# oramasearch/oramacore

Hardware: NVIDIA H100
Metric: hybrid_search_qps_at_recall10_ge_0.99_1Mx768 (higher is better)
Workload: dtype f32

## Files before the change

oramacore_b200/csrc/bm25.cuh:

```cuda
#pragma once
#include "oc_common.cuh"

namespace oc {

#ifndef OC_BM25_TILE_ROWS
#define OC_BM25_TILE_ROWS 8192
#endif
constexpr uint32_t BM25_TILE = OC_BM25_TILE_ROWS;
#ifndef OC_BM25_THREADS
#define OC_BM25_THREADS 256
#endif
constexpr uint32_t BM25_THREADS = OC_BM25_THREADS;
constexpr uint32_t BM25_CHUNK = BM25_THREADS * 4;

struct PostingRaw {
    uint32_t row;
    uint16_t tf, len;
};
struct Posting {
    uint32_t row;
    float ntf;
};

struct TermDesc {
// ... 951 lines not shown
    if (s3 != 0.f) t3_consider(s3, row + 3u, tau, tau_f, s_cnt, tbuf, cap);
}
__device__ __forceinline__ uint32_t f32_ne0_mask(const float x) {
    uint32_t r;
    asm("set.neu.u32.f32 %0, %1, 0f00000000;" : "=r"(r) : "f"(x));
    return r;
}
template <uint32_t ND, uint32_t STRIDE>
__device__ __forceinline__ void t3_scan(const float4 *d0, const float4 *d1, const float4 *d2, const float4 *d3,
                                        const uint32_t *touched, const bool any_list, const bool pos, const uint32_t row0, const uint32_t tid,
                                        const unsigned long long tau, const float tau_f, uint32_t *s_cnt, uint64_t *tbuf,
                                        const uint32_t cap, uint32_t &matched, float &lmax, float &lmin) {
    constexpr uint32_t F4 = BM25_TILE / 4 / STRIDE;
    constexpr uint32_t FB = (ND <= 2 && F4 >= 4) ? 2 : 1;
    constexpr uint32_t NB = F4 / FB;
    static_assert(F4 >= 2 && NB % 2 == 0, "tile size");
    const float4 *dp[4] = {d0, d1, d2, d3};
    const uint32_t *tw = touched + (tid >> 3);
    const uint32_t tsh = (tid & 7u) * 4u;
    float4 ca[ND][FB], cb[ND][FB];
    auto load = [&](float4 (&c)[ND][FB], const uint32_t h) {
#pragma unroll
        for (uint32_t u = 0; u < FB; u++)
#pragma unroll
            for (uint32_t d = 0; d < ND; d++) c[d][u] = __ldg(dp[d] + tid + (h * FB + u) * STRIDE);
    };
    auto fold = [&](const float4 (&c)[ND][FB], const uint32_t h) {
#pragma unroll
        for (uint32_t u = 0; u < FB; u++) {
            const uint32_t i = tid + (h * FB + u) * STRIDE;
            float sv[4] = {c[0][u].x, c[0][u].y, c[0][u].z, c[0][u].w};
#pragma unroll
            for (uint32_t d = 1; d < ND; d++) {
                sv[0] = __fadd_rn(sv[0], c[d][u].x); sv[1] = __fadd_rn(sv[1], c[d][u].y);
                sv[2] = __fadd_rn(sv[2], c[d][u].z); sv[3] = __fadd_rn(sv[3], c[d][u].w);
            }
            if (any_list) {
                const uint32_t bits = (tw[(h * FB + u) * (STRIDE / 8)] >> tsh) & 0xfu;
                if (bits) {
#pragma unroll
                    for (int k = 0; k < 4; k++) sv[k] = ((bits >> k) & 1u) ? 0.f : sv[k];
                }
            }
            matched -= f32_ne0_mask(sv[0]) + f32_ne0_mask(sv[1]) + f32_ne0_mask(sv[2]) + f32_ne0_mask(sv[3]);
            const float m4 = fmaxf(fmaxf(sv[0], sv[1]), fmaxf(sv[2], sv[3]));
            lmax = fmaxf(lmax, m4);
            if (!pos) lmin = fminf(lmin, fminf(fminf(sv[0], sv[1]), fminf(sv[2], sv[3])));
            if (m4 >= tau_f) t3_consider4(sv[0], sv[1], sv[2], sv[3], row0 + i * 4u, tau, tau_f, s_cnt, tbuf, cap);
        }
    };
    load(ca, 0);
#pragma unroll 1
    for (uint32_t h = 0; h < NB; h += 2) {
        load(cb, h + 1);
        fold(ca, h);
        if (h + 2 < NB) load(ca, h + 2);
        fold(cb, h + 1);
    }
}

__device__ __forceinline__ float t3_dense_ub(const ItemTok *tab) {
    float ub = 0.f;
#pragma unroll
    for (uint32_t j = 0; j < BM25_FLAT_TOK; j++)
        if (tab[j].n && (tab[j].flags & TD_DENSE)) ub = __fadd_rn(ub, __uint_as_float(tab[j].bound));
    return ub;
}
template <uint32_t STRIDE>
__device__ __noinline__ uint32_t t3_count(const ItemTok *tab, const uint32_t *touched, const bool any_list, const uint32_t n_tiles,
                                          const uint32_t tile, const uint32_t tid) {
    constexpr uint32_t W = BM25_TILE / 32;
    const uint32_t *bp[BM25_FLAT_TOK];
#pragma unroll
    for (uint32_t j = 0; j < BM25_FLAT_TOK; j++)
        bp[j] = (tab[j].n && (tab[j].flags & TD_DENSE))
                    ? bm25_dense_bits(reinterpret_cast<const float *>(tab[j].ptr) - size_t(tile) * BM25_TILE, n_tiles) + size_t(tile) * W
                    : nullptr;
    uint32_t m = 0;
#pragma unroll 2
    for (uint32_t w = tid; w < W; w += STRIDE) {
        uint32_t u = 0;
#pragma unroll
        for (uint32_t j = 0; j < BM25_FLAT_TOK; j++) if (bp[j]) u |= __ldg(bp[j] + w);
        if (any_list) u &= ~touched[w];
        m += __popc(u);
    }
    return m;
}

__global__ void __launch_bounds__(BM25_THREADS, 1024 / BM25_THREADS) bm25_tile3_kernel(const Bm25Params p, const ItemTok *flat, unsigned int *work_counter) {
    constexpr uint32_t W = BM25_TILE / 32;
    extern __shared__ __align__(16) uint8_t smem[];
    uint32_t *touched = reinterpret_cast<uint32_t *>(smem);
    uint32_t *bm = touched + W;
    uint64_t *tbuf = reinterpret_cast<uint64_t *>(bm + BM25_FLAT_TOK * W);
    __shared__ uint32_t s_cnt2[2], s_matched2[2];
    __shared__ unsigned int s_maxo2[2], s_mino2[2];
    __shared__ ItemTok s_tab[2][BM25_FLAT_TOK];
    __shared__ uint32_t s_item_cur, s_item_next;
    __shared__ uint32_t s_dense[2];
    __shared__ unsigned long long s_tau2[2];

    const uint32_t tid = threadIdx.x;
    const float kp1 = __fadd_rn(p.k, 1.0f);
    const uint32_t n_items = p.n_tiles * p.n_queries;
    const uint32_t *okbits = p.row_ok_bits;
// ... 130 lines not shown
            c = p.n_keep;
            if (tid == 0) atomicMax(p.tau + q, (unsigned long long)tbuf[p.n_keep - 1]);
        }
        for (uint32_t i = tid; i < c; i += BM25_THREADS) {
            const uint64_t key = tbuf[i];
            p.cand_key[slot_base * p.n_keep + i] = key;
            p.cand_ft[slot_base * p.n_keep + i] = key_score(key);
        }
        if (tid == 0) {
            p.cand_cnt[slot_base] = c;
            p.tile_count[slot_base] = s_matched2[par];
            p.tile_max[slot_base] = f32_unordered(s_maxo2[par]);
            p.tile_min[slot_base] = f32_unordered(s_mino2[par]);
        }
        if (tid < BM25_FLAT_TOK) s_tab[par ^ 1u][tid] = nx;
        if (tid == 0) { s_item_cur = next; s_item_next = next2; s_tau2[par ^ 1u] = tau_next; }
    }
    if (tid == 0 && p.dense_stat && s_dense[0]) { atomicAdd(p.dense_stat, s_dense[0]); atomicAdd(p.dense_stat + 1, s_dense[1]); }
}

constexpr uint32_t BW_WARPS = 6, BW_CAP = 256;
struct __align__(16) WarpScratch {
    uint32_t touched[BM25_TILE / 32];
    uint32_t bm[BM25_FLAT_TOK * (BM25_TILE / 32)];
    uint64_t tbuf[BW_CAP];
    ItemTok tab[BM25_FLAT_TOK];
    uint32_t cnt, dense_items, dense_skipped, pad;
};
__device__ __noinline__ unsigned long long warp_keep_top(uint64_t *buf, const uint32_t count, const uint32_t n, const uint32_t lane) {
    constexpr uint32_t PER = BW_CAP / 32;
    unsigned long long k[PER];
#pragma unroll
    for (uint32_t u = 0; u < PER; u++) k[u] = lane + 32u * u < count ? buf[lane + 32u * u] : 0ull;
    __syncwarp();
    unsigned long long mine = 0ull, last = 0ull;
    for (uint32_t r = 0; r < n; r++) {
        unsigned long long m = k[0];
#pragma unroll
        for (uint32_t u = 1; u < PER; u++) m = k[u] > m ? k[u] : m;
        for (int o = 16; o > 0; o >>= 1) {
            const unsigned long long om = __shfl_xor_sync(0xffffffffu, m, o);
            m = om > m ? om : m;
        }
        last = m;
        if (m == 0ull) break;
        if (lane == r) mine = m;
#pragma unroll
        for (uint32_t u = 0; u < PER; u++) if (k[u] == m) k[u] = 0ull;
    }
    if (lane < n) buf[lane] = mine;
    __syncwarp();
    return last;
}
__global__ void __launch_bounds__(BW_WARPS * 32, 5) bm25_warp_kernel(const Bm25Params p, const ItemTok *flat, unsigned int *work_counter) {
    constexpr uint32_t W = BM25_TILE / 32;
    extern __shared__ __align__(16) uint8_t smem[];
    const uint32_t lane = threadIdx.x & 31u;
    WarpScratch &ws = reinterpret_cast<WarpScratch *>(smem)[threadIdx.x >> 5];
    uint32_t *touched = ws.touched, *bm = ws.bm;
    const ItemTok *tab = ws.tab;
    const float kp1 = __fadd_rn(p.k, 1.0f);
    const uint32_t n_items = p.n_tiles * p.n_queries;
    const uint32_t *okbits = p.row_ok_bits;

    for (uint32_t i = lane; i < W; i += 32) touched[i] = 0u;
    for (uint32_t i = lane; i < BM25_FLAT_TOK * W; i += 32) bm[i] = 0u;
    if (lane == 0) { ws.cnt = 0u; ws.dense_items = 0u; ws.dense_skipped = 0u; }
    uint32_t item = 0, next = 0;
    if (lane == 0) { item = atomicAdd(work_counter, 1u); next = atomicAdd(work_counter, 1u); }
    item = __shfl_sync(0xffffffffu, item, 0); next = __shfl_sync(0xffffffffu, next, 0);
    ItemTok cur{};
    if (item < n_items && lane < BM25_FLAT_TOK) cur = flat[size_t(item) * BM25_FLAT_TOK + lane];
    unsigned long long tau_next = 0ull;
    if (item < n_items) tau_next = __ldcg(p.tau + item % p.n_queries);

    while (item < n_items) {
        uint32_t next2 = 0;
        if (lane == 0) next2 = atomicAdd(work_counter, 1u);
        const uint32_t tile = item / p.n_queries, q = item % p.n_queries;
        const uint32_t row0 = tile * BM25_TILE;
        if (lane < BM25_FLAT_TOK) ws.tab[lane] = cur;
        ItemTok nx{};
        if (next < n_items && lane < BM25_FLAT_TOK) nx = flat[size_t(next) * BM25_FLAT_TOK + lane];
        unsigned long long tau = __shfl_sync(0xffffffffu, tau_next, 0);
        if (next < n_items) tau_next = __ldcg(p.tau + next % p.n_queries);
        __syncwarp();

        const float4 *d0 = nullptr, *d1 = nullptr, *d2 = nullptr, *d3 = nullptr;
        uint32_t nd = 0, n_list = 0;
        bool pos = p.k >= 0.f;
#pragma unroll
        for (uint32_t j = 0; j < BM25_FLAT_TOK; j++) {
            const uint32_t n = tab[j].n;
            if (n == 0) continue;
            pos = pos && tab[j].w >= 0.f && tab[j].idf >= 0.f;
            if (tab[j].flags & TD_DENSE) {
                const float4 *dp = reinterpret_cast<const float4 *>(tab[j].ptr);
                if (nd == 0) d0 = dp; else if (nd == 1) d1 = dp; else if (nd == 2) d2 = dp; else d3 = dp;
                nd++;
            } else n_list++;
        }
        const bool any_list = n_list != 0;
        const bool use_bm = n_list > 1 || okbits != nullptr;
        uint32_t matched;
        float lmax, lmin;
        for (;;) {
            const float tau_f = tau ? key_score(tau) : -INFINITY;
            matched = 0; lmax = 0.f; lmin = 0.f;
            if (any_list && (nd || use_bm)) {
#pragma unroll 1
                for (uint32_t j = 0; j < BM25_FLAT_TOK; j++) {
                    const uint32_t n = tab[j].n;
                    if (n == 0 || (tab[j].flags & TD_DENSE)) continue;
                    const uint2 *pp = reinterpret_cast<const uint2 *>(tab[j].ptr);
                    for (uint32_t pi = lane; pi < n; pi += 32) {
                        const uint32_t row = __ldg(&pp[pi].x);
                        if (okbits && !((__ldg(okbits + (row >> 5)) >> (row & 31u)) & 1u)) continue;
                        const uint32_t l = row - row0, bit = 1u << (l & 31u);
                        if (nd) atomicOr(&touched[l >> 5], bit);
                        if (use_bm) atomicOr(&bm[j * W + (l >> 5)], bit);
                    }
                }
                __syncwarp();
            }
            const bool skip = nd && pos && t3_dense_ub(tab) < tau_f;
            if (nd && lane == 0) { ws.dense_items++; ws.dense_skipped += skip; }
            if (skip) matched += t3_count<32>(tab, touched, any_list, p.n_tiles, tile, lane);
            else switch (nd) {
                case 0: break;
                case 1: t3_scan<1, 32>(d0, d1, d2, d3, touched, any_list, pos, row0, lane, tau, tau_f, &ws.cnt, ws.tbuf, BW_CAP, matched, lmax, lmin); break;
                case 2: t3_scan<2, 32>(d0, d1, d2, d3, touched, any_list, pos, row0, lane, tau, tau_f, &ws.cnt, ws.tbuf, BW_CAP, matched, lmax, lmin); break;
                case 3: t3_scan<3, 32>(d0, d1, d2, d3, touched, any_list, pos, row0, lane, tau, tau_f, &ws.cnt, ws.tbuf, BW_CAP, matched, lmax, lmin); break;
                default: t3_scan<4, 32>(d0, d1, d2, d3, touched, any_list, pos, row0, lane, tau, tau_f, &ws.cnt, ws.tbuf, BW_CAP, matched, lmax, lmin); break;
            }
            if (any_list) {
#pragma unroll 1
                for (uint32_t j = 0; j < BM25_FLAT_TOK; j++) {
                    const uint32_t n = tab[j].n;
                    if (n == 0 || (tab[j].flags & TD_DENSE)) continue;
                    const uint2 *pp = reinterpret_cast<const uint2 *>(tab[j].ptr);
                    for (uint32_t pi = lane; pi < n; pi += 32) {
                        const uint2 rec = __ldg(pp + pi);
                        const uint32_t l = rec.x - row0, w = l >> 5, bit = 1u << (l & 31u);
                        if (use_bm) {
                            if (!(bm[j * W + w] & bit)) continue;
                            uint32_t earlier = 0;
                            for (uint32_t jj = 0; jj < j; jj++) earlier |= bm[jj * W + w];
                            if (earlier & bit) continue;
                        }
                        const float s = t3_fold(tab, bm, j, rec, l, p.k, kp1);
                        if (s != 0.f) {
                            matched++;
                            lmax = fmaxf(lmax, s);
                            lmin = fminf(lmin, s);
                            t3_consider(s, rec.x, tau, tau_f, &ws.cnt, ws.tbuf, BW_CAP);
                        }
                    }
                }
            }
            __syncwarp();
            if (any_list) {
                if (nd) for (uint32_t i = lane; i < W; i += 32) touched[i] = 0u;
                if (use_bm) for (uint32_t i = lane; i < BM25_FLAT_TOK * W; i += 32) bm[i] = 0u;
            }
            if (ws.cnt <= BW_CAP) break;
            const unsigned long long kth = warp_keep_top(ws.tbuf, BW_CAP, p.n_keep, lane) - 1ull;
            tau = kth > tau ? kth : tau;
            if (lane == 0) ws.cnt = 0u;
            __syncwarp();
        }
        matched = __reduce_add_sync(0xffffffffu, matched);
        for (int o = 16; o > 0; o >>= 1) {
            lmax = fmaxf(lmax, __shfl_xor_sync(0xffffffffu, lmax, o));
            lmin = fminf(lmin, __shfl_xor_sync(0xffffffffu, lmin, o));
        }
        const size_t slot_base = (size_t(q) * p.n_tiles + tile);
        uint32_t c = ws.cnt;
        if (c >= p.n_keep && c > 0) {
            const unsigned long long kth = warp_keep_top(ws.tbuf, c, p.n_keep, lane);
            c = p.n_keep;
            if (lane == 0) atomicMax(p.tau + q, kth);
        }
        for (uint32_t i = lane; i < c; i += 32) {
            const uint64_t key = ws.tbuf[i];
            p.cand_key[slot_base * p.n_keep + i] = key;
            p.cand_ft[slot_base * p.n_keep + i] = key_score(key);
        }
        __syncwarp();
        if (lane == 0) {
            p.cand_cnt[slot_base] = c;
            p.tile_count[slot_base] = matched;
            p.tile_max[slot_base] = lmax;
            p.tile_min[slot_base] = lmin;
            ws.cnt = 0u;
        }
        if (lane < BM25_FLAT_TOK && nx.n) {
            const char *pf = reinterpret_cast<const char *>(nx.ptr);
            const uint32_t bytes = (nx.flags & TD_DENSE) ? 1024u : min(nx.n * 8u, 1024u);
            for (uint32_t o = 0; o < bytes; o += 128u) asm volatile("prefetch.global.L1 [%0];" ::"l"(pf + o));
        }
        cur = nx;
        item = next;
        next = __shfl_sync(0xffffffffu, next2, 0);
        __syncwarp();
    }
    if (lane == 0 && p.dense_stat && ws.dense_items) { atomicAdd(p.dense_stat, ws.dense_items); atomicAdd(p.dense_stat + 1, ws.dense_skipped); }
}

struct PointParams {
    const TermDesc *terms; const TokenDesc *tokens; const QueryDesc *queries;
    uint32_t n_queries, v_stride;
    const uint32_t *v_row;
    const uint32_t *row_ok_bits;
    float k;
    int threshold;
    float *v_ft; uint8_t *v_present;
    const uint32_t *q_ok_slot;
    uint64_t ok_words;
};
__device__ __forceinline__ bool posting_find(const TermDesc &td, uint32_t row, uint32_t *payload) {
    const uint2 *pp = reinterpret_cast<const uint2 *>(td.ptr);
    uint32_t lo = 0, hi = td.len;
    while (lo < hi) { const uint32_t m = (lo + hi) >> 1; if (__ldg(&pp[m].x) < row) lo = m + 1; else hi = m; }
    if (lo < td.len) { const uint2 r = __ldg(pp + lo); if (r.x == row) { *payload = r.y; return true; } }
    return false;
}
__global__ void __launch_bounds__(256) bm25_point_kernel(const PointParams p) {
    const uint32_t wid = (blockIdx.x * blockDim.x + threadIdx.x) / 32, lane = threadIdx.x & 31;
    if (wid >= p.n_queries * p.v_stride) return;
    const uint32_t q = wid / p.v_stride;
    const uint32_t r = p.v_row[wid];
    const QueryDesc qd = p.queries[q];
    const float kp1 = __fadd_rn(p.k, 1.0f);
    float score = 0.f;
    uint32_t mask = 0;
    bool ok = r != 0xffffffffu;
    if (ok && p.row_ok_bits) ok = (row_ok_of(p.row_ok_bits, p.q_ok_slot, p.ok_words, q)[r >> 5] >> (r & 31)) & 1u;
    if (ok) {
        for (uint32_t t0 = qd.token_begin; t0 < qd.token_end; t0 += 32) {
            const uint32_t ti = t0 + lane;
            float c = __int_as_float(0x7fc00000);
            uint32_t bit = 0;
            if (ti < qd.token_end) {
                const TokenDesc tk = p.tokens[ti];
                bit = tk.bit;
                const uint32_t nt = tk.term_end - tk.term_begin;
                if (nt == 1) {
                    const TermDesc td = p.terms[tk.term_begin];
                    uint32_t pay;
                    if (td.flags & TD_DENSE) {
                        const float cd = reinterpret_cast<const float *>(td.ptr)[r];
                        if (cd != 0.f) c = cd;
                    } else if (posting_find(td, r, &pay)) {
                        if (td.flags & 1u) c = __uint_as_float(pay);
                        else {
                            const float ntf = __fmul_rn(td.weight, __uint_as_float(pay));
                            if (f32_is_normal(ntf)) c = bm25_sat(ntf, p.k, kp1, tk.idf);
                        }
                    }
// ... 96 lines not shown
```

oramacore_b200/csrc/capi.cu:

```cuda
#include <cuda_runtime.h>

#include <cub/device/device_radix_sort.cuh>
#include <cub/device/device_scan.cuh>

#include <algorithm>
#include <atomic>
#include <chrono>
#include <cmath>
#include <cstdarg>
#include <cstdio>
#include <cstring>
#include <limits>
#include <map>
#include <memory>
#include <mutex>
#include <utility>
#include <string>
#include <tuple>
#include <unordered_map>
#include <unordered_set>
#include <vector>

#include "bm25.cuh"
#include "comm.h"
// ... 89 lines not shown
    int ensure(size_t bytes) {
        if (bytes <= cap) return OC_OK;
        if (p) cudaFreeHost(p);
        p = nullptr; cap = 0;
        size_t want = bytes + bytes / 4 + 256;
        cudaError_t e = cudaMallocHost(&p, want);
        if (e != cudaSuccess) return fail(OC_ERR_OOM, "cudaMallocHost(%zu): %s", want, cudaGetErrorString(e));
        cap = want;
        return OC_OK;
    }
    template <typename T> T *as() { return reinterpret_cast<T *>(p); }
};

template <typename T> struct Slot {
    size_t off = 0;
    bool added = false;
    const T *at(const DevBuf &blob) const {
        return added ? reinterpret_cast<const T *>(static_cast<const uint8_t *>(blob.p) + off) : nullptr;
    }
};
struct Packer {
    struct Seg { const void *src; size_t off, bytes; bool direct; };
    std::vector<Seg> segs;
    size_t total = 0;
    template <typename T> Slot<T> add(const T *src, size_t n, bool direct = false) {
        const size_t off = (total + 255) & ~size_t(255);
        segs.push_back({src, off, n * sizeof(T), direct});
        total = off + n * sizeof(T);
        return Slot<T>{off, true};
    }
    void fill(void *dst) const {
        for (const Seg &g : segs) if (g.bytes && g.src && !g.direct) memcpy(static_cast<uint8_t *>(dst) + g.off, g.src, g.bytes);
    }
};
static bool is_pinned_host(const void *p) {
    cudaPointerAttributes a{};
    if (cudaPointerGetAttributes(&a, p) != cudaSuccess) { cudaGetLastError(); return false; }
    return a.type == cudaMemoryTypeHost;
}

enum { EV_START, EV_H2D, EV_DEV, EV_D2H, EV_SCAN0, EV_SCAN1, EV_BM0, EV_BM1, EV_FUSE0, EV_FUSE1, EV_COMM0, EV_COMM1, EV_SWEEP0, EV_SWEEP1, EV_RR0, EV_RR1, EV_GRP0, EV_GRP1, EV_N };

constexpr size_t P2P_WIN_BYTES = size_t(1) << 20;
constexpr uint32_t P2P_MAX_Q = 4096;
constexpr size_t P2P_FLAG_BYTES = size_t(2) * P2P_MAX_Q * 4;
constexpr uint32_t P2P_MAX_WORLD = 16;
constexpr uint32_t LOCAL_MAX_WORLD = 16;

struct oc_ctx {
    int device = 0;
    cudaStream_t stream = nullptr;
    cudaStream_t side = nullptr;
    cudaEvent_t ev_side = nullptr;
    bool sweep_timed = false;
    bool rerun_timed = false;
    bool side_dirty = false;
    cudaDeviceProp prop{};
    std::mutex mu;
    cudaEvent_t ev[EV_N]{};
    oc_timing timing{};
    uint64_t launches = 0;
    uint32_t call_launches = 0, call_scan_launches = 0;
    DevBuf in_blob, in_blob0, q_pad, q_inv, eff_norm, filter_dev, scan_cand, v_doc, v_score, v_row, v_cnt, v_srow, v_ft, v_present, v_raw;
    DevBuf seg, df_dev, row_ok, tau, cand_key, cand_ft, cand_cnt, tile_cnt, tile_max, tile_min;
    DevBuf out_blob, shard_send, shard_recv, work_ctr, flat_desc, mbits, dbits, facet_out;
    bool gemm_pending = false; const float *gemm_inv_norm = nullptr;
    DevBuf row_ft, grp_vdoc, grp_vscore, grp_vn, grp_gmin, grp_den, grp_doc, grp_score, grp_n;
    DevBuf pin_row, pin_ft, pin_ftp, pin_score, pin_present, pin_top_doc, pin_top_score, pin_top_n, pin_gdoc, pin_gscore, pin_gn;
    DevBuf srt_doc, srt_row, srt_n, srt_ft, srt_ftp, srt_score, srt_present, srt_zero;
    DevBuf mi_doc, mi_score, mi_val, mi_n, mi_cnt, mi_pscore, mi_ppresent, mi_out;
    DevBuf mg_doc, mg_score, mg_val, mg_n;
    DevBuf sfb_ws;
    DevBuf q_bf16, q_f16, q_scale, q_rho, pre_post, dense_buf, g_thr, g_eps, g_ovf, g_ovfcnt, g_resc, g_cand, g_cnt, g_flag, g_max, r_qpad, r_qinv, r_map, r_doc, r_score, r_row, r_cnt, r_raw;
    DevBuf e_rowbits, r_slot;
    const uint32_t *v_rowbits = nullptr; uint64_t v_row_words = 0;
    std::vector<uint32_t> v_qslot;
    std::vector<uint32_t> v_qlim, v_qmap;
    std::vector<float> v_qsim;
    DevBuf vq_doc, vq_score, vq_row, vq_cnt, vq_raw, r_lim, r_sim;
    DevBuf w_bits, w_blob;
    HostBuf h_where;
    DevBuf cmp_scan, cmp_stage;
    DevBuf sync_buf;
    DenseCache dense_cache;
    std::unordered_map<uint64_t, std::unique_ptr<ocdd::DictMirror>> dict_mirrors;
    DevBuf fz_in, fz_cnt, fz_out;

    HostBuf h_in, h_out, h_in0;
    OcComm comm;
    struct P2P {
        bool ready = false;
        uint8_t *local = nullptr;
        uint8_t *peer[16] = {};
        uint64_t seq = 0;
    } p2p;
    ~oc_ctx() {
        for (int r = 0; r < 16; r++) if (p2p.ready && p2p.peer[r] && p2p.peer[r] != p2p.local) cudaIpcCloseMemHandle(p2p.peer[r]);
        if (p2p.local) cudaFree(p2p.local);
        comm.destroy();
        if (stream) { dense_cache.clear(stream); cudaStreamSynchronize(stream); }
        for (int i = 0; i < EV_N; i++) if (ev[i]) cudaEventDestroy(ev[i]);
        if (stream) cudaStreamDestroy(stream);
        if (side) cudaStreamDestroy(side);
        if (ev_side) cudaEventDestroy(ev_side);
    }
};

static inline void launched(oc_ctx *c, bool scan = false) {
    c->launches++; c->call_launches++;
    if (scan) c->call_scan_launches++;
}

extern "C" int oc_init(int device_id, oc_ctx **out) {
    if (!out) return fail(OC_ERR_INVALID, "oc_init: out is NULL");
    int n = 0;
    cudaError_t e = cudaGetDeviceCount(&n);
    if (e != cudaSuccess || n == 0)
        return fail(OC_ERR_CUDA, "no CUDA device: %s (this library has no CPU fallback)", cudaGetErrorString(e));
    if (device_id < 0 || device_id >= n) return fail(OC_ERR_INVALID, "device %d out of range (%d devices)", device_id, n);
    CU(cudaSetDevice(device_id));
    oc_ctx *c = new oc_ctx();
    c->device = device_id;
    CU(cudaGetDeviceProperties(&c->prop, device_id));
    if (c->prop.major != 9 || c->prop.minor != 0) {
        int mj = c->prop.major, mn = c->prop.minor;
        delete c;
        return fail(OC_ERR_CUDA, "device sm_%d%d is not sm_90; kernels are built for sm_90a only", mj, mn);
    }
    CU(cudaStreamCreateWithFlags(&c->stream, cudaStreamNonBlocking));
    CU(cudaStreamCreateWithFlags(&c->side, cudaStreamNonBlocking));
    CU(cudaEventCreateWithFlags(&c->ev_side, cudaEventDisableTiming));
    for (int i = 0; i < EV_N; i++) CU(cudaEventCreate(&c->ev[i]));
    *out = c;
    return OC_OK;
}

extern "C" void oc_shutdown(oc_ctx *c) {
    if (!c) return;
    cudaSetDevice(c->device);
    cudaStreamSynchronize(c->stream);
    delete c;
}

extern "C" int oc_device_info(oc_ctx *c, int *sm_count, size_t *hbm_bytes, char *name, size_t name_cap) {
    if (!c) return fail(OC_ERR_INVALID, "ctx is NULL");
    if (sm_count) *sm_count = c->prop.multiProcessorCount;
    if (hbm_bytes) *hbm_bytes = c->prop.totalGlobalMem;
    if (name && name_cap) { strncpy(name, c->prop.name, name_cap - 1); name[name_cap - 1] = 0; }
    return OC_OK;
}

extern "C" int oc_pinned_alloc(size_t bytes, void **out) {
    if (!out) return fail(OC_ERR_INVALID, "out is NULL");
    CU(cudaMallocHost(out, bytes ? bytes : 1));
    return OC_OK;
}
extern "C" void oc_pinned_free(void *p) { if (p) cudaFreeHost(p); }

extern "C" int oc_last_timing(oc_ctx *c, oc_timing *out) {
    if (!c || !out) return fail(OC_ERR_INVALID, "NULL argument");
    std::lock_guard<std::mutex> g(c->mu);
    *out = c->timing;
    return OC_OK;
}
extern "C" uint64_t oc_launch_count(oc_ctx *c) { return c ? c->launches : 0; }

extern "C" int oc_comm_unique_id(uint8_t out_id[OC_COMM_ID_BYTES]) {
    std::string err;
    if (!OcComm::unique_id(out_id, &err)) return fail(OC_ERR_COMM, "%s", err.c_str());
    return OC_OK;
}
extern "C" int oc_comm_init(oc_ctx *c, int world, int rank, const uint8_t id[OC_COMM_ID_BYTES]) {
    if (!c || world < 1 || rank < 0 || rank >= world) return fail(OC_ERR_INVALID, "bad comm arguments");
    std::lock_guard<std::mutex> g(c->mu);
    CU(cudaSetDevice(c->device));
    std::string err;
    if (!c->comm.init(world, rank, id, &err)) return fail(OC_ERR_COMM, "%s", err.c_str());
    return OC_OK;
}
extern "C" int oc_comm_init_local(oc_ctx *const *ctxs, int world) {
    if (!ctxs || world < 1 || world > (int)LOCAL_MAX_WORLD) return fail(OC_ERR_INVALID, "oc_comm_init_local: 1..%u contexts", LOCAL_MAX_WORLD);
    for (int r = 0; r < world; r++) {
        if (!ctxs[r]) return fail(OC_ERR_INVALID, "oc_comm_init_local: ctxs[%d] is NULL", r);
        for (int s = 0; s < r; s++)
            if (ctxs[s] == ctxs[r]) return fail(OC_ERR_INVALID, "oc_comm_init_local: ctxs[%d] == ctxs[%d]", s, r);
    }
    auto g = std::make_shared<LocalGroup>(world);
    for (int r = 0; r < world; r++) {
// ... 3006 lines not shown
    }
    const uint32_t n_keep = k.n_keep;
    k.cap = n_keep <= 32 ? std::max<uint32_t>(n_keep + BM25_CHUNK, BM25_SPARSE_MAX)
                         : next_pow2(std::max<uint32_t>(n_keep + BM25_CHUNK, BM25_SPARSE_MAX));
    k.o_sc = size_t(B) * k.limit * 8;
    k.o_n = k.o_sc + size_t(B) * k.limit * 4;
    k.o_cnt = (k.o_n + size_t(B) * 4 + 7) & ~size_t(7);
    k.o_min = k.o_cnt + size_t(B) * 8;
    k.o_gflag = k.o_min + size_t(B) * 4;
    k.out_bytes = k.o_gflag + ((size_t(B) + 3) & ~size_t(3));
    k.o_resc = k.out_bytes + ((size_t(B) + 3) & ~size_t(3));
    k.o_dstat = k.o_resc + size_t(B) * 4;
    OCTRY(c->out_blob.ensure(k.out_bytes));
    OCTRY(c->h_out.ensure(k.o_dstat + 8));
    k.dout = c->out_blob.as<uint8_t>();
    k.d_doc = c->out_blob.as<uint64_t>();
    k.d_score = reinterpret_cast<float *>(k.dout + k.o_sc);
    k.d_n = reinterpret_cast<uint32_t *>(k.dout + k.o_n);
    return OC_OK;
}

static int bm25_stage(SearchCall &k) {
    oc_ctx *c = k.c; const oc_search_params *p = k.p;
    const uint32_t B = k.B, n_tiles = k.n_tiles, n_keep = k.n_keep; const StrSnap *S = k.S;
    const DevBuf &din = c->in_blob; cudaStream_t ps = k.side ? c->side : c->stream;
    CU(cudaEventRecord(c->ev[EV_BM0], ps));
    const uint64_t ok_words = uint64_t(n_tiles) * (BM25_TILE / 32);
    if (k.per_q) {
        OCTRY(c->row_ok.ensure(std::max<uint64_t>(ok_words, 1) * k.qfj.slots.size() * 4));
        if (ok_words) {
            rows_ok_kernel<<<dim3((unsigned)((ok_words + 255) / 256), (unsigned)k.qfj.slots.size()), 256, 0, ps>>>(
                S->row_doc, S->n_rows, k.tombs ? S->alive : nullptr, nullptr, 0, c->row_ok.as<uint32_t>(), ok_words, k.qfj.d_slots);
            launched(c);
        }
        k.row_ok = c->row_ok.as<uint32_t>();
    } else if (k.filter || k.tombs) {
        OCTRY(c->row_ok.ensure(std::max<uint64_t>(ok_words, 1) * 4));
        if (ok_words) {
            rows_ok_kernel<<<(unsigned)((ok_words + 255) / 256), 256, 0, ps>>>(
                S->row_doc, S->n_rows, k.tombs ? S->alive : nullptr, k.filter_dev, k.filter_nbits,
                c->row_ok.as<uint32_t>(), ok_words);
            launched(c);
        }
        k.row_ok = c->row_ok.as<uint32_t>();
    }
    if (!k.pre_items.empty()) {
        if (k.dense_bytes) CU(cudaMemsetAsync(c->dense_buf.p, 0, k.dense_bytes, ps));
        for (const DenseEntry *e : k.dense_new) CU(cudaMemsetAsync(e->p, 0, e->bytes, ps));
        bm25_precompute_kernel<<<(unsigned)k.pre_items.size(), 256, 0, ps>>>(k.s_pre.at(din), k.s_pitems.at(din), p->bm25_k, k.row_ok);
        launched(c);
        CU(cudaGetLastError());
        for (DenseEntry *e : k.dense_new) e->ready = true;
    }
    const size_t n_td = k.terms.size();
    OCTRY(c->seg.ensure((n_td * (size_t(n_tiles) + 1) + 1) * 4));
    if (n_td) {
        const uint64_t work = uint64_t(n_td) * (n_tiles + 1);
        bm25_plan_kernel<<<(unsigned)((work + 255) / 256), 256, 0, ps>>>(k.s_terms.at(din), (uint32_t)n_td, n_tiles, c->seg.as<uint32_t>());
        launched(c);
    }
    if (k.need_df) {
        const size_t ntok = k.tokens.size();
        OCTRY(c->df_dev.ensure(ntok * 4));
        CU(cudaMemsetAsync(c->df_dev.p, 0, ntok * 4, c->stream));
        DfParams dp{};
        dp.terms = k.s_terms.at(din);
        dp.tokens = k.s_tokens.at(din);
        dp.n_tokens = (uint32_t)ntok; dp.n_tiles = n_tiles; dp.seg = c->seg.as<uint32_t>();
        dp.row_ok_bits = k.row_ok; dp.df = c->df_dev.as<unsigned int>();
        if (k.per_q) { dp.tok_ok_slot = k.s_tslot.at(din); dp.ok_words = ok_words; }
        if (n_tiles && ntok) {
            bm25_df_kernel<<<(unsigned)(uint64_t(n_tiles) * ntok), BM25_THREADS, 0, c->stream>>>(dp);
            launched(c);
        }
        if (k.multi_rank) {
            std::string err;
            if (!c->comm.all_reduce_sum_u32(c->df_dev.p, c->df_dev.p, ntok, c->stream, &err)) return fail(OC_ERR_COMM, "%s", err.c_str());
        }
        std::vector<uint32_t> dfh(ntok);
        CU(cudaMemcpyAsync(dfh.data(), c->df_dev.p, ntok * 4, cudaMemcpyDeviceToHost, c->stream));
        CU(cudaStreamSynchronize(c->stream));
        const float N = (float)S->document_count;
        for (size_t t = 0; t < ntok; t++)
            if (k.tok_need_df[t]) k.tokens[t].idf = host_idf(N, std::max<uint32_t>(1u, dfh[t]));
        CU(cudaMemcpyAsync(const_cast<TokenDesc *>(k.s_tokens.at(din)), k.tokens.data(), ntok * sizeof(TokenDesc),
                           cudaMemcpyHostToDevice, c->stream));
    }
    const size_t slots = size_t(B) * std::max<uint32_t>(n_tiles, 1);
    OCTRY(c->tau.ensure(size_t(B) * 16 + 16));
    OCTRY(c->cand_key.ensure(slots * n_keep * 8));
    OCTRY(c->cand_ft.ensure(slots * n_keep * 4));
    OCTRY(c->cand_cnt.ensure(slots * 4));
    OCTRY(c->tile_cnt.ensure(slots * 4));
    OCTRY(c->tile_max.ensure(slots * 4));
    OCTRY(c->tile_min.ensure(slots * 4));
    k.min_hint_dev = reinterpret_cast<float *>(c->tau.as<uint8_t>() + size_t(B) * 8);
    k.tile_counter = reinterpret_cast<unsigned int *>(c->tau.as<uint8_t>() + size_t(B) * 16);
    CU(cudaMemsetAsync(c->tau.p, 0, size_t(B) * 16 + 16, ps));
    Bm25Params &bp = k.bp;
    bp.terms = k.s_terms.at(din);
    bp.tokens = k.s_tokens.at(din);
    bp.queries = k.s_queries.at(din);
    bp.term_token = k.s_ttok.at(din);
    bp.seg = c->seg.as<uint32_t>();
    bp.n_queries = B; bp.n_tiles = n_tiles; bp.n_rows = S->n_rows;
    bp.k = p->bm25_k;
    bp.row_ok_bits = k.row_ok;
    if (k.per_q) { bp.q_ok_slot = k.qfj.d_q_slot_ft; bp.ok_words = ok_words; }
    bp.omc_row = p->omc ? k.omc_row_dev : k.s_omcr.at(din);
    bp.omc_mult = p->omc ? k.omc_row_mult_dev : k.s_omcrm.at(din);
    bp.n_omc = k.n_omc_rows;
    bp.min_hint = k.min_hint_dev;
    bp.n_keep = n_keep; bp.cap = k.cap;
    bp.tau = c->tau.as<unsigned long long>();
    bp.cand_key = c->cand_key.as<uint64_t>(); bp.cand_ft = c->cand_ft.as<float>();
    bp.cand_cnt = c->cand_cnt.as<uint32_t>(); bp.tile_count = c->tile_cnt.as<uint32_t>();
    bp.tile_max = c->tile_max.as<float>(); bp.tile_min = c->tile_min.as<float>();
    bp.dense_stat = k.tile_counter + 2;
    const SearchReq &r = k.r;
    if (r.fj || r.gj || r.sj) {
        OCTRY(c->mbits.ensure(size_t(B) * std::max<uint32_t>(n_tiles, 1) * (BM25_TILE / 32) * 4));
        bp.matched_bits = c->mbits.as<uint32_t>();
    }
    if (r.gj && n_tiles) {
        OCTRY(c->row_ft.ensure(size_t(B) * n_tiles * BM25_TILE * 4));
        bp.row_ft = c->row_ft.as<float>();
    }
    if (n_tiles) OCTRY(launch_tile(c, bp, n_tiles * B, k.any_multi, k.thr, k.omc_tile, ps, k.max_tokens, k.tile_counter, k.need_df));
    CU(cudaEventRecord(c->ev[EV_BM1], ps));
    c->timing.bm25_postings = k.postings_walked;
    if (k.side) {
        CU(cudaEventRecord(c->ev_side, c->side));
        CU(cudaStreamWaitEvent(c->stream, c->ev_side, 0));
        c->side_dirty = false;
    }
    return OC_OK;
}

static void point_lookup(SearchCall &k, const uint32_t *rows, uint32_t stride, float *out_ft, uint8_t *out_present, uint64_t n_slots) {
    PointParams pp{};
    pp.terms = k.bp.terms; pp.tokens = k.bp.tokens; pp.queries = k.bp.queries;
    pp.n_queries = k.B; pp.v_stride = stride; pp.v_row = rows; pp.row_ok_bits = k.row_ok;
    pp.q_ok_slot = k.per_q ? k.qfj.d_q_slot_ft : nullptr; pp.ok_words = uint64_t(k.n_tiles) * (BM25_TILE / 32);
    pp.k = k.p->bm25_k; pp.threshold = k.thr ? 1 : 0;
    pp.v_ft = out_ft; pp.v_present = out_present;
    bm25_point_kernel<<<(unsigned)((n_slots * 32 + 255) / 256), 256, 0, k.c->stream>>>(pp);
    launched(k.c);
}

static void pin_scores(SearchCall &k, uint32_t stride, const uint64_t *doc, const uint32_t *cnt, const float *ft,
                       const uint8_t *ft_present, float *out_score, uint8_t *out_present) {
    const FuseParams &fp = k.fp;
    PinScoreParams sp{};
    sp.n_queries = k.B; sp.stride = stride; sp.doc = doc; sp.cnt = cnt;
    sp.has_ft = k.has_ft; sp.hybrid = k.has_ft && k.has_v;
    sp.ft = ft; sp.ft_present = ft_present;
    sp.gmin = fp.out_gmin; sp.den = fp.out_den;
    sp.v_doc = fp.out_vdoc; sp.v_score = fp.out_vscore; sp.v_n = fp.out_vn; sp.v_stride = std::max<uint32_t>(k.vlimit, 1);
    sp.omc_doc = fp.omc_doc; sp.omc_mult = fp.omc_mult; sp.n_omc = k.n_omc;
    sp.out_score = out_score; sp.out_present = out_present;
    sp.q_plan = k.s_plan.at(k.c->in_blob);
    pin_score_kernel<<<(unsigned)((uint64_t(k.B) * stride * 32 + 255) / 256), 256, 0, k.c->stream>>>(sp);
    launched(k.c);
}

static int pin_tail(SearchCall &k) {
    if (!k.pin_items) return OC_OK;
    oc_ctx *c = k.c; const PinJob *pj = k.r.pj;
    const uint32_t B = k.B, ps = pj->stride;
    const uint64_t nslot = uint64_t(B) * ps;
    OCTRY(c->pin_score.ensure(nslot * 4));
    OCTRY(c->pin_present.ensure(nslot));
    if (k.has_ft) {
        OCTRY(c->pin_row.ensure(nslot * 4));
        OCTRY(c->pin_ft.ensure(nslot * 4));
        OCTRY(c->pin_ftp.ensure(nslot));
        map_docs_to_rows_kernel<<<(unsigned)((nslot + 255) / 256), 256, 0, c->stream>>>(
            pj->d_doc, pj->d_cnt, ps, B, k.S->row_doc, k.S->n_rows, c->pin_row.as<uint32_t>());
        launched(c);
        point_lookup(k, c->pin_row.as<uint32_t>(), ps, c->pin_ft.as<float>(), c->pin_ftp.as<uint8_t>(), nslot);
    }
    pin_scores(k, ps, pj->d_doc, pj->d_cnt, c->pin_ft.as<float>(), c->pin_ftp.as<uint8_t>(), c->pin_score.as<float>(),
               c->pin_present.as<uint8_t>());
    if (k.pin_flat) {
        PinSpliceParams xp{};
        xp.stride = ps; xp.kp2 = std::max<uint32_t>(32, next_pow2(ps));
        xp.doc = pj->d_doc; xp.pos = pj->d_pos; xp.score = c->pin_score.as<float>(); xp.cnt = pj->d_cnt;
        xp.n_top = k.n_keep; xp.limit = k.limit; xp.offset = k.p->offset;
// ... 43 lines not shown
    if (pj->splice) {
        xp.stride = pj->stride; xp.kp2 = std::max<uint32_t>(32, next_pow2(pj->stride));
        xp.doc = pj->d_doc; xp.pos = pj->d_pos; xp.score = c->pin_score.as<float>(); xp.cnt = pj->d_cnt;
    } else {
        OCTRY(c->srt_zero.ensure(size_t(B) * 4));
        CU(cudaMemsetAsync(c->srt_zero.p, 0, size_t(B) * 4, c->stream));
        xp.stride = 0; xp.kp2 = 32;
        xp.doc = c->srt_doc.as<uint64_t>(); xp.pos = c->srt_zero.as<uint32_t>(); xp.score = c->srt_score.as<float>();
        xp.cnt = c->srt_zero.as<uint32_t>();
    }
    xp.n_top = top; xp.limit = limit; xp.offset = offset;
    xp.top_doc = c->srt_doc.as<uint64_t>(); xp.top_score = c->srt_score.as<float>(); xp.top_n = c->srt_n.as<uint32_t>();
    xp.out_doc = k.d_doc; xp.out_score = k.d_score; xp.out_n = k.d_n;
    if (sj->by_score) {
        xp.q_alt = k.s_salt.at(din); xp.alt_n_top = n_keep;
        xp.alt_doc = c->pin_top_doc.as<uint64_t>(); xp.alt_score = c->pin_top_score.as<float>(); xp.alt_n = c->pin_top_n.as<uint32_t>();
    }
    xp.q_page = k.s_page.at(din);
    pin_splice_kernel<<<B, PIN_THREADS, pin_splice_smem(xp.kp2, sj->by_score ? std::max(top, n_keep) : top, k.qp ? k.page_max : limit + offset),
                        c->stream>>>(xp);
    launched(c);
    CU(cudaGetLastError());
    return OC_OK;
}

static int fuse_and_tails(SearchCall &k) {
    void (*fuse)(const FuseParams) = k.exports ? fuse_topk_kernel<true> : fuse_topk_kernel<false>;
    fuse<<<k.B, 256, k.fuse_smem, k.c->stream>>>(k.fp);
    launched(k.c);
    CU(cudaGetLastError());
    OCTRY(pin_tail(k));
    return sort_tail(k);
}

static int fuse_or_merge(SearchCall &k) {
    oc_ctx *c = k.c;
    if (!(k.p->sharded && c->comm.world > 1)) return fuse_and_tails(k);
    const bool has_v = k.has_v;
    OCTRY(run_sharded_merge(c, k.p, k.fp, k.has_ft ? (uint32_t)k.S->n_rows : 0, has_v ? (uint32_t)k.emb->n_rows : 0, k.B,
                            (has_v && c->gemm_pending) ? c->g_flag.as<uint8_t>() : nullptr, k.dout + k.o_gflag));
    k.did_comm = true;
    return OC_OK;
}

static int device_tail(SearchCall &k) {
    oc_ctx *c = k.c; const oc_search_params *p = k.p;
    const uint32_t B = k.B, vlimit = k.vlimit, n_keep = k.n_keep; const bool has_ft = k.has_ft, has_v = k.has_v;
    const StrSnap *S = k.S;
    if (has_ft && has_v) {
        OCTRY(c->v_srow.ensure(size_t(B) * vlimit * 4));
        OCTRY(c->v_ft.ensure(size_t(B) * vlimit * 4));
        OCTRY(c->v_present.ensure(size_t(B) * vlimit));
        if (vlimit) {
            map_docs_to_rows_kernel<<<(B * vlimit + 255) / 256, 256, 0, c->stream>>>(
                c->v_doc.as<uint64_t>(), c->v_cnt.as<uint32_t>(), vlimit, B, S->row_doc, S->n_rows, c->v_srow.as<uint32_t>());
            launched(c);
            point_lookup(k, c->v_srow.as<uint32_t>(), vlimit, c->v_ft.as<float>(), c->v_present.as<uint8_t>(), uint64_t(B) * vlimit);
            CU(cudaGetLastError());
        }
    }
    FuseParams &fp = k.fp;
    fp = FuseParams{};
    fp.mode = k.mode; fp.n_tiles = k.n_tiles; fp.n_keep = n_keep; fp.limit = k.limit; fp.offset = p->offset;
    fp.q_plan = k.s_plan.at(c->in_blob);
    {
        const uint64_t total = (has_ft ? uint64_t(k.n_tiles) * n_keep : 0) + (has_v ? vlimit : 0);
        fp.capb = next_pow2((uint32_t)std::min<uint64_t>(16384, std::max<uint64_t>(total, 2 * n_keep)));
        fp.capb = std::max<uint32_t>(fp.capb, std::max<uint32_t>(64, next_pow2(2 * n_keep)));
    }
    if (has_ft) {
        const Bm25Params &bp = k.bp;
        fp.cand_key = bp.cand_key; fp.cand_ft = bp.cand_ft; fp.cand_cnt = bp.cand_cnt; fp.tile_count = bp.tile_count;
        fp.tile_max = bp.tile_max; fp.tile_min = bp.tile_min; fp.str_row_doc_ids = S->row_doc;
    }
    if (has_v) {
        fp.v_doc = c->v_doc.as<uint64_t>(); fp.v_score = c->v_score.as<float>(); fp.v_count = c->v_cnt.as<uint32_t>();
        fp.v_row = has_ft ? c->v_srow.as<uint32_t>() : nullptr;
        fp.v_ft = c->v_ft.as<float>(); fp.v_present = c->v_present.as<uint8_t>();
    }
    fp.v_stride = vlimit;
    fp.omc_doc = p->omc ? k.omc_doc : k.s_omcd.at(c->in_blob);
    fp.omc_mult = p->omc ? k.omc_mult : k.s_omcm.at(c->in_blob);
    fp.n_omc = k.n_omc;
    fp.out_doc = k.d_doc; fp.out_score = k.d_score; fp.out_n = k.d_n;
    fp.out_count = reinterpret_cast<unsigned long long *>(k.dout + k.o_cnt);
    fp.out_min = reinterpret_cast<float *>(k.dout + k.o_min);
    if (k.k4_top) {
        fp.limit = n_keep; fp.offset = 0;
        OCTRY(c->pin_top_doc.ensure(size_t(B) * n_keep * 8));
        OCTRY(c->pin_top_score.ensure(size_t(B) * n_keep * 4));
        OCTRY(c->pin_top_n.ensure(size_t(B) * 4));
        fp.out_doc = c->pin_top_doc.as<uint64_t>(); fp.out_score = c->pin_top_score.as<float>(); fp.out_n = c->pin_top_n.as<uint32_t>();
    }
    if (k.exports) {
        const uint32_t vs = std::max<uint32_t>(vlimit, 1);
        OCTRY(c->grp_vdoc.ensure(size_t(B) * vs * 8));
        OCTRY(c->grp_vscore.ensure(size_t(B) * vs * 4));
        OCTRY(c->grp_vn.ensure(size_t(B) * 4));
        OCTRY(c->grp_gmin.ensure(size_t(B) * 4));
        OCTRY(c->grp_den.ensure(size_t(B) * 4));
        fp.out_vdoc = c->grp_vdoc.as<uint64_t>(); fp.out_vscore = c->grp_vscore.as<float>(); fp.out_vn = c->grp_vn.as<uint32_t>();
        fp.out_gmin = c->grp_gmin.as<float>(); fp.out_den = c->grp_den.as<float>();
    }
    k.fuse_smem = size_t(fp.capb) * 8 + size_t(std::max<uint32_t>(32, next_pow2(n_keep))) * 8 + size_t(vlimit) * 16 + 64;
    const void *fuse = k.exports ? (const void *)fuse_topk_kernel<true> : (const void *)fuse_topk_kernel<false>;
    CU(smem_cfg(c->device, fuse, k.fuse_smem));
    CU(cudaEventRecord(c->ev[EV_FUSE0], c->stream));
    OCTRY(fuse_or_merge(k));
    CU(cudaEventRecord(c->ev[EV_FUSE1], c->stream));
    return OC_OK;
}

// ... 2706 lines not shown
```

Before: 174,500.

## Overlap vector point lookup with side-stream BM25 and early-exit dense scan on overflow

The main stream now waits only on an earlier side-stream event before running the vector-to-row mapping and point lookup, and defers the full side-stream join until just before fusion. This lets the point lookup overlap the BM25 tile kernel instead of serializing after it. The dense scan loop also exits early once the candidate buffer overflows its cap, skipping useless work before the re-threshold pass. Compile-gated per-phase profiling instrumentation is added as well. The risk is a subtle race if the point lookup depends on any side-stream output produced after the new early event.

```diff
diff --git a/oramacore_b200/csrc/bm25.cuh b/oramacore_b200/csrc/bm25.cuh
--- a/oramacore_b200/csrc/bm25.cuh
+++ b/oramacore_b200/csrc/bm25.cuh
@@ -1027,6 +1027,7 @@
     load(ca, 0);
 #pragma unroll 1
     for (uint32_t h = 0; h < NB; h += 2) {
+        if (h && *reinterpret_cast<volatile const uint32_t *>(s_cnt) > cap) break;
         load(cb, h + 1);
         fold(ca, h);
         if (h + 2 < NB) load(ca, h + 2);
@@ -1263,6 +1264,25 @@
     __syncwarp();
     return last;
 }
+enum { BWP_DESC, BWP_MARK, BWP_DENSE, BWP_FOLD, BWP_CLEAR, BWP_KEEP, BWP_EMIT, BWP_N };
+struct BwProfItem {
+    uint32_t item, cls;
+    uint32_t postings, cand;
+    uint32_t span[BWP_N];
+    uint32_t smid;
+};
+struct BwProfWarp { unsigned long long t0, t1, c0, c1; uint32_t smid, items, pad[2]; };
+struct BwProf { BwProfItem *items; BwProfWarp *warps; unsigned int *n_items, *n_warps; uint32_t cap_items, cap_warps; };
+#ifdef OC_BM25_PHASE_PROFILE
+__device__ BwProf g_bw_prof;
+__device__ __forceinline__ unsigned long long bw_gtime() { unsigned long long t; asm volatile("mov.u64 %0, %%globaltimer;" : "=l"(t)); return t; }
+__device__ __forceinline__ uint32_t bw_smid() { uint32_t s; asm volatile("mov.u32 %0, %%smid;" : "=r"(s)); return s; }
+#define BW_PROF(...) __VA_ARGS__
+#define BW_LAP(ph) do { const long long t_ = clock64(); pspan[ph] += uint32_t(t_ - pclk); pclk = t_; } while (0)
+#else
+#define BW_PROF(...)
+#define BW_LAP(ph) do { } while (0)
+#endif
 __global__ void __launch_bounds__(BW_WARPS * 32, 5) bm25_warp_kernel(const Bm25Params p, const ItemTok *flat, unsigned int *work_counter) {
     constexpr uint32_t W = BM25_TILE / 32;
     extern __shared__ __align__(16) uint8_t smem[];
@@ -1284,8 +1304,10 @@
     if (item < n_items && lane < BM25_FLAT_TOK) cur = flat[size_t(item) * BM25_FLAT_TOK + lane];
     unsigned long long tau_next = 0ull;
     if (item < n_items) tau_next = __ldcg(p.tau + item % p.n_queries);
+    BW_PROF(const unsigned long long prof_t0 = bw_gtime(), prof_c0 = clock64(); uint32_t prof_items = 0;)
 
     while (item < n_items) {
+        BW_PROF(uint32_t pspan[BWP_N] = {}; long long pclk = clock64(); uint32_t prof_passes = 0, prof_skip = 0, prof_post = 0;)
         uint32_t next2 = 0;
         if (lane == 0) next2 = atomicAdd(work_counter, 1u);
         const uint32_t tile = item / p.n_queries, q = item % p.n_queries;
@@ -1309,15 +1331,17 @@
                 const float4 *dp = reinterpret_cast<const float4 *>(tab[j].ptr);
                 if (nd == 0) d0 = dp; else if (nd == 1) d1 = dp; else if (nd == 2) d2 = dp; else d3 = dp;
                 nd++;
-            } else n_list++;
+            } else { n_list++; BW_PROF(prof_post += n;) }
         }
         const bool any_list = n_list != 0;
         const bool use_bm = n_list > 1 || okbits != nullptr;
         uint32_t matched;
         float lmax, lmin;
+        BW_LAP(BWP_DESC);
         for (;;) {
             const float tau_f = tau ? key_score(tau) : -INFINITY;
             matched = 0; lmax = 0.f; lmin = 0.f;
+            BW_PROF(prof_passes++;)
             if (any_list && (nd || use_bm)) {
 #pragma unroll 1
                 for (uint32_t j = 0; j < BM25_FLAT_TOK; j++) {
@@ -1334,8 +1358,10 @@
                 }
                 __syncwarp();
             }
+            BW_LAP(BWP_MARK);
             const bool skip = nd && pos && t3_dense_ub(tab) < tau_f;
             if (nd && lane == 0) { ws.dense_items++; ws.dense_skipped += skip; }
+            BW_PROF(prof_skip = skip;)
             if (skip) matched += t3_count<32>(tab, touched, any_list, p.n_tiles, tile, lane);
             else switch (nd) {
                 case 0: break;
@@ -1344,6 +1370,7 @@
                 case 3: t3_scan<3, 32>(d0, d1, d2, d3, touched, any_list, pos, row0, lane, tau, tau_f, &ws.cnt, ws.tbuf, BW_CAP, matched, lmax, lmin); break;
                 default: t3_scan<4, 32>(d0, d1, d2, d3, touched, any_list, pos, row0, lane, tau, tau_f, &ws.cnt, ws.tbuf, BW_CAP, matched, lmax, lmin); break;
             }
+            BW_LAP(BWP_DENSE);
             if (any_list) {
 #pragma unroll 1
                 for (uint32_t j = 0; j < BM25_FLAT_TOK; j++) {
@@ -1370,15 +1397,18 @@
                 }
             }
             __syncwarp();
+            BW_LAP(BWP_FOLD);
             if (any_list) {
                 if (nd) for (uint32_t i = lane; i < W; i += 32) touched[i] = 0u;
                 if (use_bm) for (uint32_t i = lane; i < BM25_FLAT_TOK * W; i += 32) bm[i] = 0u;
             }
+            BW_LAP(BWP_CLEAR);
             if (ws.cnt <= BW_CAP) break;
             const unsigned long long kth = warp_keep_top(ws.tbuf, BW_CAP, p.n_keep, lane) - 1ull;
             tau = kth > tau ? kth : tau;
             if (lane == 0) ws.cnt = 0u;
             __syncwarp();
+            BW_LAP(BWP_KEEP);
         }
         matched = __reduce_add_sync(0xffffffffu, matched);
         for (int o = 16; o > 0; o >>= 1) {
@@ -1387,11 +1417,14 @@
         }
         const size_t slot_base = (size_t(q) * p.n_tiles + tile);
         uint32_t c = ws.cnt;
+        BW_PROF(const uint32_t prof_cand = c;)
+        BW_LAP(BWP_EMIT);
         if (c >= p.n_keep && c > 0) {
             const unsigned long long kth = warp_keep_top(ws.tbuf, c, p.n_keep, lane);
             c = p.n_keep;
             if (lane == 0) atomicMax(p.tau + q, kth);
         }
+        BW_LAP(BWP_KEEP);
         for (uint32_t i = lane; i < c; i += 32) {
             const uint64_t key = ws.tbuf[i];
             p.cand_key[slot_base * p.n_keep + i] = key;
@@ -1410,12 +1443,32 @@
             const uint32_t bytes = (nx.flags & TD_DENSE) ? 1024u : min(nx.n * 8u, 1024u);
             for (uint32_t o = 0; o < bytes; o += 128u) asm volatile("prefetch.global.L1 [%0];" ::"l"(pf + o));
         }
+        BW_LAP(BWP_EMIT);
+        BW_PROF(if (lane == 0 && g_bw_prof.n_items) {
+            const BwProf &g = g_bw_prof;
+            const uint32_t s = atomicAdd(g.n_items, 1u);
+            if (s < g.cap_items) {
+                BwProfItem &r = g.items[s];
+                r.item = item; r.cls = nd | n_list << 4 | prof_skip << 8 | prof_passes << 12;
+                r.postings = prof_post; r.cand = prof_cand; r.smid = bw_smid();
+                for (int ph = 0; ph < BWP_N; ph++) r.span[ph] = pspan[ph];
+            }
+            prof_items++;
+        })
         cur = nx;
         item = next;
         next = __shfl_sync(0xffffffffu, next2, 0);
         __syncwarp();
     }
     if (lane == 0 && p.dense_stat && ws.dense_items) { atomicAdd(p.dense_stat, ws.dense_items); atomicAdd(p.dense_stat + 1, ws.dense_skipped); }
+    BW_PROF(if (lane == 0 && g_bw_prof.n_warps) {
+        const BwProf &g = g_bw_prof;
+        const uint32_t s = atomicAdd(g.n_warps, 1u);
+        if (s < g.cap_warps) {
+            BwProfWarp &r = g.warps[s];
+            r.t0 = prof_t0; r.t1 = bw_gtime(); r.c0 = prof_c0; r.c1 = clock64(); r.smid = bw_smid(); r.items = prof_items;
+        }
+    })
 }
 
 struct PointParams {
diff --git a/oramacore_b200/csrc/capi.cu b/oramacore_b200/csrc/capi.cu
--- a/oramacore_b200/csrc/capi.cu
+++ b/oramacore_b200/csrc/capi.cu
@@ -165,6 +165,7 @@
     cudaStream_t stream = nullptr;
     cudaStream_t side = nullptr;
     cudaEvent_t ev_side = nullptr;
+    cudaEvent_t ev_side_in = nullptr;
     bool sweep_timed = false;
     bool rerun_timed = false;
     bool side_dirty = false;
@@ -216,6 +217,7 @@
         if (stream) cudaStreamDestroy(stream);
         if (side) cudaStreamDestroy(side);
         if (ev_side) cudaEventDestroy(ev_side);
+        if (ev_side_in) cudaEventDestroy(ev_side_in);
     }
 };
 
@@ -243,10 +245,22 @@
     CU(cudaStreamCreateWithFlags(&c->stream, cudaStreamNonBlocking));
     CU(cudaStreamCreateWithFlags(&c->side, cudaStreamNonBlocking));
     CU(cudaEventCreateWithFlags(&c->ev_side, cudaEventDisableTiming));
+    CU(cudaEventCreateWithFlags(&c->ev_side_in, cudaEventDisableTiming));
     for (int i = 0; i < EV_N; i++) CU(cudaEventCreate(&c->ev[i]));
     *out = c;
     return OC_OK;
 }
+
+#ifdef OC_BM25_PHASE_PROFILE
+extern "C" int oc_bm25_phase_profile(void *items, uint32_t cap_items, void *warps, uint32_t cap_warps, void *counters) {
+    BwProf g{};
+    g.items = static_cast<BwProfItem *>(items); g.warps = static_cast<BwProfWarp *>(warps);
+    g.n_items = static_cast<unsigned int *>(counters); g.n_warps = g.n_items + 1;
+    g.cap_items = cap_items; g.cap_warps = cap_warps;
+    CU(cudaMemcpyToSymbol(g_bw_prof, &g, sizeof(g)));
+    return OC_OK;
+}
+#endif
 
 extern "C" void oc_shutdown(oc_ctx *c) {
     if (!c) return;
@@ -3359,6 +3373,7 @@
         CU(cudaGetLastError());
         for (DenseEntry *e : k.dense_new) e->ready = true;
     }
+    if (k.side) CU(cudaEventRecord(c->ev_side_in, c->side));
     const size_t n_td = k.terms.size();
     OCTRY(c->seg.ensure((n_td * (size_t(n_tiles) + 1) + 1) * 4));
     if (n_td) {
@@ -3436,11 +3451,7 @@
     if (n_tiles) OCTRY(launch_tile(c, bp, n_tiles * B, k.any_multi, k.thr, k.omc_tile, ps, k.max_tokens, k.tile_counter, k.need_df));
     CU(cudaEventRecord(c->ev[EV_BM1], ps));
     c->timing.bm25_postings = k.postings_walked;
-    if (k.side) {
-        CU(cudaEventRecord(c->ev_side, c->side));
-        CU(cudaStreamWaitEvent(c->stream, c->ev_side, 0));
-        c->side_dirty = false;
-    }
+    if (k.side) CU(cudaEventRecord(c->ev_side, c->side));
     return OC_OK;
 }
 
@@ -3590,12 +3601,17 @@
         OCTRY(c->v_ft.ensure(size_t(B) * vlimit * 4));
         OCTRY(c->v_present.ensure(size_t(B) * vlimit));
         if (vlimit) {
+            if (k.side) CU(cudaStreamWaitEvent(c->stream, c->ev_side_in, 0));
             map_docs_to_rows_kernel<<<(B * vlimit + 255) / 256, 256, 0, c->stream>>>(
                 c->v_doc.as<uint64_t>(), c->v_cnt.as<uint32_t>(), vlimit, B, S->row_doc, S->n_rows, c->v_srow.as<uint32_t>());
             launched(c);
             point_lookup(k, c->v_srow.as<uint32_t>(), vlimit, c->v_ft.as<float>(), c->v_present.as<uint8_t>(), uint64_t(B) * vlimit);
             CU(cudaGetLastError());
         }
+    }
+    if (k.side) {
+        CU(cudaStreamWaitEvent(c->stream, c->ev_side, 0));
+        c->side_dirty = false;
     }
     FuseParams &fp = k.fp;
     fp = FuseParams{};
```

New measurement: 187,300, median of 6. 7.3% higher.
